# jzhangbs/MVSDF

Measured on AMD Instinct MI355X. Metric: traced rays/sec (fwd+bwd, 10 sphere iters, 4 src views), higher is better.
Workload: dtype f32x3

## Files before the change

mvsdf_amd/csrc/step_driver.hip:

```cpp
#include <hip/hip_runtime.h>
#include <stdint.h>
#include <stdlib.h>
#include <string.h>
#include <new>
#include "capi_util.h"
#include "step_internal.h"
#include <sched.h>
#include <time.h>

namespace {

inline size_t al256(size_t x) { return (x + 255) & ~(size_t)255; }

struct FwdOffsets {
    size_t w[MVSDF_STEP_MAX_LAYERS], wp[MVSDF_STEP_MAX_LAYERS], wpT[MVSDF_STEP_MAX_LAYERS], wp16[MVSDF_STEP_MAX_LAYERS];
    size_t wx3[MVSDF_STEP_MAX_LAYERS], wx3T[MVSDF_STEP_MAX_LAYERS];
    int chain_x3;
    size_t trace_ws, trace_ws_bytes;
    size_t inv, true_rows, true_rank, counts, view_sorted;
    size_t x_eval, y_eval, n_eval, sdf_ctx, rgb_sorted, render_ctx;
};
struct BwdOffsets {
    size_t dy, dn, dy_x, dn_x, din, drgb_sorted, render_ws, wsA, wsX, dx, fbar;
};

struct Step {
    MvsdfStepDesc d;
    MvsdfStepLayout lay;
    FwdOffsets fo;
    BwdOffsets bo;
    int R, E, M, Nout, K0r, nl;
    size_t woff[MVSDF_STEP_MAX_LAYERS], boff[MVSDF_STEP_MAX_LAYERS];
    size_t seg[2][3];
    long long* counts_host;
    long long* counts_host_dev;
    int can_defer;
    hipEvent_t ev_counts;
    bool counts_pending;
    long long counts_seq;
    hipStream_t counts_stream;
    int timing;
    hipEvent_t ev_t[9];
    bool timed, timed_bwd;
    hipStream_t side;
    hipEvent_t ev_fork, ev_join;
    int split_rows;
};

void make_descs(const Step& st, const MvsdfStepParams* prm, const char* fwd, MvsdfNetDesc* sdf, MvsdfNetDesc* sdfT, MvsdfNetDesc* rnd, MvsdfNetDesc* rndT) {
    const MvsdfStepDesc& d = st.d;
    auto fill = [&](MvsdfNetDesc* o, MvsdfNetDesc* oT, int l0, int n, bool is_sdf) {
        memset(o, 0, sizeof(*o));
        memset(oT, 0, sizeof(*oT));
        o->n_layers = oT->n_layers = n;
        for (int i = 0; i < n; ++i) {
            const int l = l0 + i;
            o->K[i] = d.K[l]; o->N[i] = d.N[l];
            oT->K[i] = d.N[l]; oT->N[i] = d.K[l];
            o->wp[i] = (const float*)(fwd + st.fo.wp[l]);
            oT->wp[i] = (const float*)(fwd + st.fo.wpT[l]);
            o->bias[i] = oT->bias[i] = prm->b[l];
            o->w[i] = oT->w[i] = (const float*)(fwd + st.fo.w[l]);
            if (is_sdf && d.trace_dtype != 0) o->wp16[i] = fwd + st.fo.wp16[l];
            if (is_sdf && st.fo.chain_x3) { o->wx3[i] = fwd + st.fo.wx3[l]; oT->wx3[i] = fwd + st.fo.wx3T[l]; }
        }
        if (is_sdf) {
            const unsigned m = d.skip_mask;
            const int single = (m && !(m & (m - 1))) ? __builtin_ctz(m) : -1;
            o->skip_layer = oT->skip_layer = m ? (single >= 0 ? single : __builtin_ctz(m)) : -1;
            o->skip_mask = (m && single < 0) ? m : 0;
            o->multires = oT->multires = d.multires;
            o->trace_dtype = (d.trace_dtype >= 1 && d.trace_dtype <= 5) ? d.trace_dtype : 0;
        } else {
            o->skip_layer = oT->skip_layer = -1;
        }
    };
    fill(sdf, sdfT, 0, d.n_sdf, true);
    fill(rnd, rndT, d.n_sdf, d.n_render, false);
}

__global__ void k_step_gather_x(const float* __restrict__ eik, int n_eik, const float* __restrict__ ds_on, const float* __restrict__ ds_jit, int n_ds,
                                const float* __restrict__ points, const long long* __restrict__ perm, int R, float* __restrict__ x_eval,
                                uint8_t* __restrict__ ones) {
    const int E = n_eik + 2 * n_ds, total = (E + R) * 3;
    for (int i = blockIdx.x * blockDim.x + threadIdx.x; i < total; i += gridDim.x * blockDim.x) {
        const int row = i / 3, c = i - 3 * row;
        float v;
        if (row < n_eik) v = eik[i];
        else if (row < n_eik + n_ds) v = ds_on[3 * (size_t)(row - n_eik) + c];
        else if (row < E) v = ds_jit[3 * (size_t)(row - n_eik - n_ds) + c];
        else v = points[3 * (size_t)perm[row - E] + c];
        x_eval[i] = v;
        if (ones && i < R) ones[i] = 1;
    }
}

__global__ void k_step_gather_drgb(const float* __restrict__ d_rgb, const long long* __restrict__ perm, int N, float* __restrict__ out) {
    const int i = blockIdx.x * blockDim.x + threadIdx.x;
    if (i >= 3 * N) return;
    const int row = i / 3, c = i - 3 * row;
    out[i] = d_rgb[3 * (size_t)perm[row] + c];
}

#define ST_TRY(expr) do { int rc_ = (expr); if (rc_) return rc_; } while (0)
#define ST_HIP(expr) do { hipError_t e_ = (expr); if (e_ != hipSuccess) return mv_check(e_, #expr); } while (0)

}

extern "C" {

int mvsdf_step_create(const MvsdfStepDesc* desc, MvsdfStepLayout* layout, void** out) {
    if (!desc || !layout || !out) return mv_fail(-1, "mvsdf_step_create: null argument");
    if (desc->trace_dtype == 1) return mv_fail(-2, "mvsdf_step_create: trace_dtype 1 (bf16 weights AND 8-bit activations) was removed in round 5: use 3 (bf16x2)");
    const MvsdfStepDesc& d = *desc;
    const int nl = d.n_sdf + d.n_render;
    if (d.B <= 0 || d.P <= 0 || d.n_eik < 0 || d.n_ds < 0 || d.n_sdf < 2 || d.n_render < 1 || d.n_sdf > MVSDF_MAX_LAYERS || d.n_render > MVSDF_MAX_LAYERS ||
        nl > MVSDF_STEP_MAX_LAYERS || (long long)d.B * d.P > (1ll << 24))
        return mv_fail(-1, "mvsdf_step_create: bad sizes");
    Step* st = new (std::nothrow) Step;
    if (!st) return mv_fail(-1, "mvsdf_step_create: out of host memory");
    memset(st, 0, sizeof(*st));
    st->d = d;
    st->R = d.B * d.P; st->E = d.n_eik + 2 * d.n_ds; st->M = st->R + st->E; st->nl = nl;
    st->Nout = d.N[d.n_sdf - 1]; st->K0r = d.K[d.n_sdf];
    st->split_rows = -1;
    const int R = st->R, M = st->M;
    MvsdfNetDesc sdf, sdfT, rnd, rndT;
    MvsdfStepParams fake;
    memset(&fake, 0, sizeof(fake));
    static const float dummy = 0.f;
    for (int l = 0; l < nl; ++l) fake.b[l] = &dummy;
    MvsdfStepLayout& L = st->lay;
    FwdOffsets& fo = st->fo;
    size_t p = 0;
    auto take = [&](size_t bytes) { const size_t o = p; p += al256(bytes ? bytes : 4); return o; };
    L.ray_dirs = take((size_t)R * 12); L.cam_loc = take((size_t)d.B * 12);
    L.points = take((size_t)R * 12); L.mask = take((size_t)R); L.dists = take((size_t)R * 4); L.counters = take(16 * 8);
    L.object_mask_out = take((size_t)R);
    fo.trace_ws_bytes = mvsdf_trace_workspace_bytes_n(R, d.tp.n_steps);
    fo.trace_ws = take(fo.trace_ws_bytes);
    fo.chain_x3 = mv_chain_x3_enabled();
    for (int l = 0; l < nl; ++l) {
        fo.w[l] = take((size_t)d.N[l] * d.K[l] * 4);
        fo.wp[l] = take(mvsdf_packed_floats(d.N[l], d.K[l]) * 4);
        fo.wpT[l] = take(mvsdf_packed_floats(d.K[l], d.N[l]) * 4);
        if (l < d.n_sdf && d.trace_dtype == 2) {
            fo.wp16[l] = take(mvsdf_packed_floats(d.N[l], d.K[l]) * 4);
        } else if (l < d.n_sdf && (d.trace_dtype == 3 || d.trace_dtype == 4)) {
            fo.wp16[l] = take(mvsdf_packed_bf16_bytes(d.N[l], d.K[l], 0));
        } else if (l < d.n_sdf && d.trace_dtype == 5) {
            fo.wp16[l] = take(3 * mvsdf_packed_bf16_bytes(d.N[l], d.K[l], 0));
        }
        if (l < d.n_sdf && fo.chain_x3) {
            fo.wx3[l] = d.trace_dtype == 5 ? fo.wp16[l] : take(3 * mvsdf_packed_bf16_bytes(d.N[l], d.K[l], 0));
            fo.wx3T[l] = take(3 * mvsdf_packed_bf16_bytes(d.K[l], d.N[l], 0));
        }
    }
    L.perm = take((size_t)R * 8); fo.inv = take((size_t)R * 8); fo.true_rows = take((size_t)R * 8); fo.true_rank = take((size_t)R * 4); fo.counts = take(4 * 8 + 4 * 4);
    fo.view_sorted = take((size_t)R * 12);
    fo.x_eval = take((size_t)M * 12); fo.y_eval = take((size_t)M * st->Nout * 4); fo.n_eval = take((size_t)M * 12);
    make_descs(*st, &fake, (const char*)nullptr, &sdf, &sdfT, &rnd, &rndT);
    for (int i = 0; i < d.n_sdf; ++i) { sdf.wp[i] = sdfT.wp[i] = &dummy; sdf.w[i] = &dummy; }
    for (int i = 0; i < d.n_render; ++i) { rnd.wp[i] = rndT.wp[i] = &dummy; }
    const size_t ctx_f = mvsdf_sdf_ctx_floats(&sdf, M, M), rctx_f = mvsdf_render_ctx_floats(&rnd, R);
    if (!ctx_f || !rctx_f) { delete st; return mv_fail(-2, "mvsdf_step_create: network descriptor rejected (layer dims / skip mask)"); }
    st->can_defer = (d.n_ds == 0 && mv_step_can_defer(&sdf, &sdfT, &rnd, &rndT)) ? 1 : 0;
    fo.sdf_ctx = take(ctx_f * 4);
    fo.rgb_sorted = take((size_t)R * 12);
    fo.render_ctx = take(rctx_f * 4);
    L.rgb_values = take((size_t)R * 12); L.sdf_output = take((size_t)R * 4); L.diff_pts = take((size_t)R * 12);
    L.eik_out = take((size_t)M * 4); L.points_hom = take((size_t)M * 16); L.grad_theta = take((size_t)M * 12);
    L.surf = take((size_t)(R + d.n_eik) * 4);
    L.fwd_bytes = p;
    BwdOffsets& bo = st->bo;
    p = 0;
    bo.dy = take((size_t)M * st->Nout * 4); bo.dn = take((size_t)M * 12);
    bo.dy_x = take((size_t)R * st->Nout * 4); bo.dn_x = take((size_t)R * 12);
    bo.din = take((size_t)R * st->K0r * 4); bo.drgb_sorted = take((size_t)R * 12);
    bo.render_ws = take(mvsdf_render_bwd_ws_floats(&rnd, R) * 4);
    bo.wsA = take(mvsdf_sdf_bwd_ws_floats(&sdf, M) * 4);
    bo.wsX = take(mvsdf_sdf_bwd_ws_floats(&sdf, R) * 4);
    bo.dx = take((size_t)R * 12); bo.fbar = take((size_t)R * 4);
    size_t off = 0;
    int lo = 0;
    const int cuts[2] = {d.n_sdf, nl};
    for (int net = 0; net < 2; ++net) {
        st->seg[net][0] = off;
        for (int l = lo; l < cuts[net]; ++l) { st->woff[l] = off; off += (size_t)d.N[l] * d.K[l]; }
        st->seg[net][1] = off;
        for (int l = lo; l < cuts[net]; ++l) { st->boff[l] = off; off += (size_t)d.N[l]; }
        st->seg[net][2] = off;
        lo = cuts[net];
    }
    L.dflat_floats = off;
    L.dflat = take(off * 4);
    L.bwd_bytes = p;
    *layout = L;
    *out = st;
    return 0;
}

void mvsdf_step_destroy(void* step) {
    Step* st = (Step*)step;
    if (!st) return;
    if (st->timing) for (int i = 0; i < 9; ++i) hipEventDestroy(st->ev_t[i]);
    if (st->counts_host) { hipEventDestroy(st->ev_counts); hipHostFree(st->counts_host); }
    if (st->side) { hipStreamSynchronize(st->side); hipEventDestroy(st->ev_fork); hipEventDestroy(st->ev_join); hipStreamDestroy(st->side); }
    delete st;
}

int mvsdf_step_set_timing(void* step, int enable) {
    Step* st = (Step*)step;
    if (!st) return mv_fail(-1, "mvsdf_step_set_timing: null step");
    if (enable && !st->timing) {
        for (int i = 0; i < 9; ++i) ST_HIP(hipEventCreate(&st->ev_t[i]));
        st->timing = 1;
    } else if (!enable && st->timing) {
        for (int i = 0; i < 9; ++i) hipEventDestroy(st->ev_t[i]);
        st->timing = 0;
    }
    st->timed = false; st->timed_bwd = false;
    return 0;
}

int mvsdf_step_trace_times(void* step, float ms[3]) {
    Step* st = (Step*)step;
    if (!st || !ms || !st->timing || !st->timed) return mv_fail(-1, "mvsdf_step_trace_times: timing is off or no forward has run");
    float a = 0.f, b = 0.f, c = 0.f;
    ST_HIP(hipEventElapsedTime(&a, st->ev_t[0], st->ev_t[1]));
    ST_HIP(hipEventElapsedTime(&b, st->ev_t[1], st->ev_t[2]));
    ST_HIP(hipEventElapsedTime(&c, st->ev_t[3], st->ev_t[4]));
    ms[0] = a; ms[1] = b; ms[2] = c;
    return 0;
}

int mvsdf_step_times(void* step, float ms[6]) {
    Step* st = (Step*)step;
    if (!st || !ms || !st->timing || !st->timed) return mv_fail(-1, "mvsdf_step_times: timing is off or no forward has run");
    if (int rc = mvsdf_step_trace_times(step, ms)) return rc;
    ST_HIP(hipEventElapsedTime(&ms[3], st->ev_t[4], st->ev_t[5]));
    ms[4] = 0.f;
    if (st->timed_bwd) ST_HIP(hipEventElapsedTime(&ms[4], st->ev_t[6], st->ev_t[7]));
    ST_HIP(hipEventElapsedTime(&ms[5], st->ev_t[8], st->ev_t[5]));
    return 0;
}

int mvsdf_step_forward(void* step, const MvsdfStepParams* prm, const MvsdfStepInputs* in, int d_mask, int e_mask, void* fwd_, void* stream) {
    Step* st = (Step*)step;
    if (!st || !prm || !in || !fwd_) return mv_fail(-1, "mvsdf_step_forward: null argument");
    const MvsdfStepDesc& d = st->d;
    if (!in->uv || !in->pose || !in->intrinsics || !in->object_mask || !in->object_mask_true || !in->intervals || !in->minsdf_steps ||
        (d.n_eik > 0 && !in->eik_points) || (d.n_ds > 0 && (!in->ds_on || !in->ds_jit || !in->ds_counts)))
        return mv_fail(-1, "mvsdf_step_forward: missing input");
    hipStream_t s = (hipStream_t)stream;
    if (!st->counts_host) {
        ST_HIP(hipHostMalloc((void**)&st->counts_host, MVSDF_STEP_COUNT_RING * 8 * sizeof(long long), hipHostMallocMapped | hipHostMallocCoherent));
        memset(st->counts_host, 0, MVSDF_STEP_COUNT_RING * 8 * sizeof(long long));
        if (hipHostGetDevicePointer((void**)&st->counts_host_dev, st->counts_host, 0) != hipSuccess) { (void)hipGetLastError(); st->counts_host_dev = nullptr; }
        if (hipEventCreateWithFlags(&st->ev_counts, hipEventDisableTiming) != hipSuccess) {
            hipHostFree(st->counts_host); st->counts_host = nullptr;
            return mv_fail(-1, "mvsdf_step_forward: hipEventCreate failed");
        }
    }
    char* fwd = (char*)fwd_;
    const MvsdfStepLayout& L = st->lay;
    const FwdOffsets& fo = st->fo;
    const int R = st->R, E = st->E, M = st->M, nl = st->nl;
    if (st->timing) ST_HIP(hipEventRecord(st->ev_t[8], s));
    float* w[MVSDF_STEP_MAX_LAYERS]; float* wp[MVSDF_STEP_MAX_LAYERS]; float* wpT[MVSDF_STEP_MAX_LAYERS];
    for (int l = 0; l < nl; ++l) { w[l] = (float*)(fwd + fo.w[l]); wp[l] = (float*)(fwd + fo.wp[l]); wpT[l] = (float*)(fwd + fo.wpT[l]); }
    float* ray_dirs = (float*)(fwd + L.ray_dirs); float* cam_loc = (float*)(fwd + L.cam_loc);
    {
        void* wp16[MVSDF_STEP_MAX_LAYERS]; int nsplit[MVSDF_STEP_MAX_LAYERS];
        void* wx3[MVSDF_STEP_MAX_LAYERS]; void* wx3T[MVSDF_STEP_MAX_LAYERS];
        for (int l = 0; l < nl; ++l) {
            const bool bf = l < d.n_sdf && d.trace_dtype != 0;
            wp16[l] = bf ? (void*)(fwd + fo.wp16[l]) : nullptr;
            const bool x3 = l < d.n_sdf && fo.chain_x3;
            wx3[l] = (x3 && d.trace_dtype != 5) ? (void*)(fwd + fo.wx3[l]) : nullptr;
            wx3T[l] = x3 ? (void*)(fwd + fo.wx3T[l]) : nullptr;
            nsplit[l] = 0;
        }
        const float* stage_dev = nullptr;
        if (in->host_stage) {
            if (hipHostGetDevicePointer((void**)&stage_dev, (void*)in->host_stage, 0) != hipSuccess || !stage_dev) {
                (void)hipGetLastError();
                return mv_fail(-1, "mvsdf_step_forward: host_stage is not device-visible pinned memory");
            }
        }
        ST_TRY(mv_step_prologue(nl, prm->v, prm->g, d.N, d.K, w, wp, wpT, wp16, nsplit, d.trace_dtype == 2 ? 1 : (d.trace_dtype == 5 ? 2 : 0), wx3, wx3T, in->uv, in->pose, in->intrinsics, d.B, d.P, ray_dirs, cam_loc,
                                (uint8_t*)(fwd + L.object_mask_out), (unsigned long long*)(fwd + L.counters), stage_dev, (float*)in->minsdf_steps, d.tp.n_steps,
                                (float*)in->eik_points, 3 * d.n_eik, stream));
    }
    MvsdfNetDesc sdf, sdfT, rnd, rndT;
    make_descs(*st, prm, fwd, &sdf, &sdfT, &rnd, &rndT);
    float* x_eval = (float*)(fwd + fo.x_eval); float* y_eval = (float*)(fwd + fo.y_eval); float* n_eval = (float*)(fwd + fo.n_eval);
    FwdGather g;
    g.eik = in->eik_points; g.on = in->ds_on; g.jit = in->ds_jit; g.pts = (float*)(fwd + L.points); g.perm = (long long*)(fwd + L.perm);
    g.n_eik = d.n_eik; g.n_ds = d.n_ds; g.x_out = x_eval;
    if (st->split_rows < 0) {
        const char* e = getenv("MVSDF_SPLIT_ROWS");
        st->split_rows = (e && *e) ? (atoi(e) != 0 && E >= 1) : mv_chain_split_pays(&sdf, E, M);
        if (st->split_rows) {
            int prio_least = 0, prio_greatest = 0;
            if (hipDeviceGetStreamPriorityRange(&prio_least, &prio_greatest) != hipSuccess) { (void)hipGetLastError(); prio_least = 0; }
            if (hipStreamCreateWithPriority(&st->side, hipStreamNonBlocking, prio_least) != hipSuccess) { (void)hipGetLastError(); st->side = nullptr; st->split_rows = 0; }
            else if (hipEventCreateWithFlags(&st->ev_fork, hipEventDisableTiming) != hipSuccess ||
                     hipEventCreateWithFlags(&st->ev_join, hipEventDisableTiming) != hipSuccess) {
                (void)hipGetLastError();
                if (st->ev_fork) { (void)hipEventDestroy(st->ev_fork); st->ev_fork = nullptr; }
                if (st->ev_join) { (void)hipEventDestroy(st->ev_join); st->ev_join = nullptr; }
                (void)hipStreamDestroy(st->side);
                st->side = nullptr; st->split_rows = 0;
            }
        }
    }
    bool split = st->split_rows == 1;
    struct SideGuard {
        hipStream_t side; bool armed;
        ~SideGuard() { if (armed && side) (void)hipStreamSynchronize(side); }
    } side_guard{st->side, false};
    if (split) ST_HIP(hipEventRecord(st->ev_fork, s));
    float* points = (float*)(fwd + L.points); uint8_t* mask = (uint8_t*)(fwd + L.mask); float* dists = (float*)(fwd + L.dists);
    unsigned long long* counters = (unsigned long long*)(fwd + L.counters);
    auto stage = [&](int which) {
        return mvsdf_trace_stage(which, &sdf, &d.tp, cam_loc, ray_dirs, in->object_mask, d.B, d.P, 1, in->intervals, in->minsdf_steps, points, mask, dists,
                                 counters, fwd + fo.trace_ws, fo.trace_ws_bytes, d.mt, d.mt_samples, stream);
    };
    if (st->timing) ST_HIP(hipEventRecord(st->ev_t[0], s));
    ST_TRY(mv_trace_stage1_prezeroed(&sdf, &d.tp, cam_loc, ray_dirs, in->object_mask, d.B, d.P, 1, in->intervals, in->minsdf_steps, points, mask, dists,
                                     counters, fwd + fo.trace_ws, fo.trace_ws_bytes, d.mt, d.mt_samples, stream));
    if (st->timing) ST_HIP(hipEventRecord(st->ev_t[1], s));
    if (split) {
        ST_HIP(hipStreamWaitEvent(st->side, st->ev_fork, 0));
        side_guard.armed = true;
        const int rcs = mv_sdf_forward_gather(&sdf, &sdfT, nullptr, &g, M, M, 0, E, y_eval, n_eval, (float*)(fwd + fo.sdf_ctx), st->side);
        if (rcs == 1) { split = false; side_guard.armed = false; }
        else if (rcs) return rcs;
        else ST_HIP(hipEventRecord(st->ev_join, st->side));
    }
    ST_TRY(stage(3));
    if (st->timing) ST_HIP(hipEventRecord(st->ev_t[2], s));
    long long* perm = (long long*)(fwd + L.perm); long long* inv = (long long*)(fwd + fo.inv); long long* true_rows = (long long*)(fwd + fo.true_rows);
    long long* counts = (long long*)(fwd + fo.counts); float* view_sorted = (float*)(fwd + fo.view_sorted);
    ST_TRY(mv_partition_rays_step(mask, d.use_object_mask ? in->object_mask : nullptr, in->object_mask_true, ray_dirs, R, perm, inv, true_rows, counts,
                                  view_sorted, (int*)(fwd + fo.true_rank), d.n_ds > 0 ? in->ds_counts : nullptr,
                                  st->counts_host_dev ? st->counts_host_dev + 8 * ((st->counts_seq + 1) % MVSDF_STEP_COUNT_RING) : nullptr, st->counts_seq + 1,
                                  (float*)(fwd + fo.counts + 32), d.n_eik, d.n_ds, d_mask, e_mask, stream));
    ++st->counts_seq;
    if (!st->counts_host_dev) {
        ST_HIP(hipMemcpyAsync(st->counts_host, counts, 4 * sizeof(long long), hipMemcpyDeviceToHost, s));
        ST_HIP(hipEventRecord(st->ev_counts, s));
    }
    st->counts_pending = true; st->counts_stream = s;
    if (st->timing) ST_HIP(hipEventRecord(st->ev_t[3], s));
    ST_TRY(stage(4));
    if (st->timing) { ST_HIP(hipEventRecord(st->ev_t[4], s)); st->timed = true; }
    {
        if (split) { ST_HIP(hipStreamWaitEvent(s, st->ev_join, 0)); side_guard.armed = false; }
        int rcf = mv_sdf_forward_gather(&sdf, &sdfT, nullptr, &g, M, M, split ? E : 0, M, y_eval, n_eval, (float*)(fwd + fo.sdf_ctx), stream);
        if (rcf == 1) {
            const int total = M * 3;
            hipLaunchKernelGGL(k_step_gather_x, dim3((total + 255) / 256), dim3(256), 0, s, in->eik_points, d.n_eik, in->ds_on, in->ds_jit, d.n_ds, points, perm,
                               R, x_eval, (uint8_t*)nullptr);
            ST_HIP(hipGetLastError());
            rcf = mvsdf_sdf_forward(&sdf, &sdfT, x_eval, M, M, y_eval, n_eval, (float*)(fwd + fo.sdf_ctx), stream);
        }
        if (rcf) return rcf;
    }
    float* rgb_sorted = (float*)(fwd + fo.rgb_sorted);
    ST_TRY(mvsdf_render_forward(&rnd, x_eval + 3 * (size_t)E, view_sorted, n_eval + 3 * (size_t)E, y_eval + (size_t)E * st->Nout + 2, st->Nout, R,
                                d.view_spec, rgb_sorted, (float*)(fwd + fo.render_ctx), stream));
    ST_TRY(mvsdf_step_outputs(R, d.n_eik, d.n_ds, st->Nout, counts, x_eval, y_eval, n_eval, inv, true_rows, rgb_sorted, d_mask, e_mask,
                              (float*)(fwd + L.rgb_values), (float*)(fwd + L.sdf_output), (float*)(fwd + L.diff_pts), (float*)(fwd + L.eik_out),
                              (float*)(fwd + L.points_hom), (float*)(fwd + L.grad_theta), (float*)(fwd + L.surf), stream));
    if (st->timing) ST_HIP(hipEventRecord(st->ev_t[5], s));
    return 0;
}

static int step_wait_seq(Step* st, long long seq, long long counts[4]) {
    long long* slot = st->counts_host + 8 * (seq % MVSDF_STEP_COUNT_RING);
    for (unsigned long long it = 1;; ++it) {
        const long long have = __atomic_load_n(&slot[4], __ATOMIC_ACQUIRE);
        if (have == seq) break;
        if (have > seq) return mv_fail(-4, "mvsdf_step_wait_counts_seq: the record of that forward was overwritten (read the counts from its forward block)");
        if (it < 5000) { __builtin_ia32_pause(); continue; }
        struct timespec ts = {0, 20000};
        nanosleep(&ts, nullptr);
        if ((it & 0x3ff) == 0 && seq == st->counts_seq) {
            const hipError_t q = hipStreamQuery(st->counts_stream);
            if (q == hipSuccess) {
                if (__atomic_load_n(&slot[4], __ATOMIC_ACQUIRE) == seq) break;
                return mv_fail(-1, "mvsdf_step_wait_counts: the forward finished without delivering its counts");
            }
            if (q != hipErrorNotReady) return mv_check(q, "mvsdf_step_wait_counts (hipStreamQuery)");
        }
    }
    for (int i = 0; i < 4; ++i) counts[i] = slot[i];
    if (__atomic_load_n(&slot[4], __ATOMIC_ACQUIRE) != seq) return mv_fail(-4, "mvsdf_step_wait_counts_seq: the record of that forward was overwritten (read the counts from its forward block)");
    return 0;
}

int mvsdf_step_wait_counts(void* step, long long counts[4]) {
    Step* st = (Step*)step;
    if (!st || !counts) return mv_fail(-1, "mvsdf_step_wait_counts: null argument");
    if (!st->counts_pending) return mv_fail(-1, "mvsdf_step_wait_counts: no forward is in flight");
    if (!st->counts_host_dev) {
        ST_HIP(hipEventSynchronize(st->ev_counts));
        for (int i = 0; i < 4; ++i) counts[i] = st->counts_host[i];
        st->counts_pending = false;
        return 0;
    }
    const int rc = step_wait_seq(st, st->counts_seq, counts);
    st->counts_pending = false;
    return rc;
}

long long mvsdf_step_seq(void* step) { return step ? ((Step*)step)->counts_seq : -1; }
size_t mvsdf_step_counts_offset(void* step) { return step ? ((Step*)step)->fo.counts : 0; }
int mvsdf_step_can_defer(void* step) { Step* st = (Step*)step; return (st && st->can_defer) ? 1 : 0; }
int mvsdf_step_saved_offsets(void* step, size_t out[6]) {
    Step* st = (Step*)step;
    if (!st || !out) return mv_fail(-1, "mvsdf_step_saved_offsets: null argument");
    out[0] = st->fo.x_eval; out[1] = st->fo.y_eval; out[2] = st->fo.n_eval; out[3] = st->fo.view_sorted; out[4] = st->fo.render_ctx; out[5] = st->fo.rgb_sorted;
    return 0;
}

int mvsdf_step_wait_counts_seq(void* step, long long seq, long long counts[4]) {
    Step* st = (Step*)step;
    if (!st || !counts) return mv_fail(-1, "mvsdf_step_wait_counts_seq: null argument");
    if (seq <= 0 || seq > st->counts_seq || !st->counts_host) return mv_fail(-1, "mvsdf_step_wait_counts_seq: no such forward");
    if (!st->counts_host_dev) {
        if (seq != st->counts_seq) return mv_fail(-4, "mvsdf_step_wait_counts_seq: the record of that forward was overwritten (read the counts from its forward block)");
        ST_HIP(hipEventSynchronize(st->ev_counts));
        for (int i = 0; i < 4; ++i) counts[i] = st->counts_host[i];
        return 0;
    }
    if (seq + MVSDF_STEP_COUNT_RING <= st->counts_seq) return mv_fail(-4, "mvsdf_step_wait_counts_seq: the record of that forward was overwritten (read the counts from its forward block)");
    const int rc = step_wait_seq(st, seq, counts);
    if (rc == 0 && seq == st->counts_seq) st->counts_pending = false;
    return rc;
}
// ... 139 lines not shown
```

mvsdf_amd/csrc/trace.hip:

```cpp
#include <stdlib.h>
#include <type_traits>
#include "tile_engine.h"
#include "tile_engine_bf16.h"
#include "tile_engine_bf16s.h"
#include "trace_params.h"
#include "capi_util.h"

struct RayCommon {
    float c[3], d[3];
};

__device__ __forceinline__ float mv_clamp(float v, float lo, float hi) { return v < lo ? lo : (v > hi ? hi : v); }

__device__ __forceinline__ bool mv_sphere_isect(const float* c, const float* d, float r, float& t0, float& t1) {
    const float dot = fmaf(d[2], c[2], fmaf(d[1], c[1], d[0] * c[0]));
    const float nrm = sqrtf(c[0] * c[0] + c[1] * c[1] + c[2] * c[2]);
    const float under = dot * dot - (nrm * nrm - r * r);
    const bool hit = under > 0.0f;
    float a = 0.0f, b = 0.0f;
    if (hit) {
        const float s = sqrtf(under);
        a = s * -1.0f - dot;
        b = s * 1.0f - dot;
    }
// ... 425 lines not shown
        const int kind = e >> 28;
        const bool om = kind & MV_ITEM_OM;
        cc = c.cam_loc + 3 * (gid / c.P);
        d = c.dirs + 3 * (size_t)gid;
        const float zmin = c.w_zmin[gid], zmax = c.w_zmax[gid];
        const int row = src ? src[it] : it;
        const float* sv = c.sv + (size_t)row * n_steps;
        if (mode == 0 && c.n_first < n_steps) {
            if (it == 0 && lead) {
                atomicAdd(&c.counters[MV_CNT_ROWS_SAMPLER], (unsigned long long)n_list * (unsigned long long)n_steps);
                atomicAdd(&c.counters[MV_CNT_ROWS_SAMPLER_EVAL], (unsigned long long)n_list * (unsigned long long)c.n_first);
            }
            const int ind = mv_first_where(sv, c.n_first, lane, 0);
            if (!(om && ind >= 1)) {
                cat = 1;
            } else if (lead) {
                dist = zmin + c.intervals[ind] * (zmax - zmin);
                have_dist = true;
                c.o_mask[gid] = 1;
                cat = 2;
                c.sec_state[gid] = zmin + c.intervals[ind - 1] * (zmax - zmin);
                c.sec_state[(size_t)c.R + gid] = dist;
                c.sec_state[2 * (size_t)c.R + gid] = sv[ind - 1];
                c.sec_state[3 * (size_t)c.R + gid] = sv[ind];
            }
        } else if (mode <= 1) {
            if (it == 0 && lead) {
                if (mode == 0) {
                    atomicAdd(&c.counters[MV_CNT_ROWS_SAMPLER], (unsigned long long)n_list * (unsigned long long)n_steps);
                    atomicAdd(&c.counters[MV_CNT_ROWS_SAMPLER_EVAL], (unsigned long long)n_list * (unsigned long long)n_steps);
                } else
                    atomicAdd(&c.counters[MV_CNT_ROWS_SAMPLER_EVAL], (unsigned long long)n_list * (unsigned long long)(n_steps - c.n_first));
            }
            int ind = mv_first_where(sv, n_steps, lane, 0);
            if (ind < 0) ind = mv_first_where(sv, n_steps, lane, 1);
            if (ind < 0) ind = n_steps - 1;
            const bool net_surf = sv[ind] < 0.f;
            const int i2 = (om && net_surf) ? 0 : mv_first_argmin(sv, n_steps, lane);
            if (lead) {
                dist = zmin + c.intervals[(om && net_surf) ? ind : i2] * (zmax - zmin);
                have_dist = true;
                c.o_mask[gid] = net_surf ? 1 : 0;
                const bool do_secant = c.training ? (net_surf && om) : net_surf;
                if (do_secant) {
                    int lo = ind - 1; if (lo < 0) lo += n_steps;
                    cat = 2;
                    c.sec_state[gid] = zmin + c.intervals[lo] * (zmax - zmin);
                    c.sec_state[(size_t)c.R + gid] = zmin + c.intervals[ind] * (zmax - zmin);
                    c.sec_state[2 * (size_t)c.R + gid] = sv[lo];
                    c.sec_state[3 * (size_t)c.R + gid] = sv[ind];
                }
            }
        } else {
            if (it == 0 && lead) atomicAdd(&c.counters[MV_CNT_ROWS_MINSDF], (unsigned long long)n_list * (unsigned long long)n_steps);
            const int bi = mv_first_argmin(sv, n_steps, lane);
            if (lead) { dist = c.steps[bi] * (zmax - zmin) + zmin; have_dist = true; }
        }
        if (lead && have_dist) {
            c.o_dists[gid] = dist;
            c.o_points[3 * (size_t)gid + 0] = cc[0] + dist * d[0];
            c.o_points[3 * (size_t)gid + 1] = cc[1] + dist * d[1];
            c.o_points[3 * (size_t)gid + 2] = cc[2] + dist * d[2];
        }
    }
    if (mode == 2) return;
    if (lead) s_cat[w] = cat;
    __syncthreads();
    if (threadIdx.x == 0) {
        unsigned n1 = 0, n2 = 0;
        for (int k = 0; k < MV_RED_WAVES; ++k) { n1 += s_cat[k] == 1; n2 += s_cat[k] == 2; }
        if (n1) s_base[0] = atomicAdd(&c.counters[MV_CNT_N_SAMPLER_REST], (unsigned long long)n1);
        if (n2) s_base[1] = atomicAdd(&c.counters[MV_CNT_N_SECANT], (unsigned long long)n2);
    }
    __syncthreads();
    if (lead && cat) {
        unsigned rank = 0;
        for (int k = 0; k < w; ++k) rank += s_cat[k] == cat;
        const unsigned long long k = s_base[cat - 1] + rank;
        if (cat == 1) { c.list_rest[k] = e; c.src_rest[k] = it; }
        else c.sec_list[k] = gid;
    }
}

template <int MT, int NTW, int NW, class NET>
__device__ void mv_secant_rays(const NET& net, const MvTraceParams& tp, const SampleCtx& c, int n_list, int block, float* smem) {
    constexpr int ROWS = 16 * MT;
    const int tid = threadIdx.x;
    const int r0 = block * ROWS;
    if (r0 >= n_list) return;
    const int n = min(ROWS, n_list - r0);
    TraceLds lds = mv_carve<NET>(smem, ROWS, net.S, 3 + 6 * net.multires, 0);
    const bool mine = tid < n;
    int gid = 0;
    float cc[3] = {0, 0, 0}, d[3] = {0, 0, 0}, z_low = 0, z_high = 0, sdf_low = 0, sdf_high = 1, z_pred = 0;
    if (mine) {
        gid = c.sec_list[r0 + tid];
        const int b = gid / c.P;
        for (int i = 0; i < 3; ++i) { cc[i] = c.cam_loc[3 * b + i]; d[i] = c.dirs[3 * (size_t)gid + i]; }
        z_low = c.sec_state[gid]; z_high = c.sec_state[(size_t)c.R + gid];
        sdf_low = c.sec_state[2 * (size_t)c.R + gid]; sdf_high = c.sec_state[3 * (size_t)c.R + gid];
        z_pred = -sdf_low * (z_high - z_low) / (sdf_high - sdf_low) + z_low;
    }
    for (int it = 0; it < tp.n_secant; ++it) {
        if (tid < ROWS) { float* p = lds.pts + tid * 3; p[0] = cc[0] + z_pred * d[0]; p[1] = cc[1] + z_pred * d[1]; p[2] = cc[2] + z_pred * d[2]; }
        __syncthreads();
        mv_eval_dispatch<MT, NTW, NW>(net, (n + 15) >> 4, lds.act, lds.pe, lds.pts, lds.sdfv, tid);
        if (mine) {
            const float sm = lds.sdfv[tid];
            if (sm > 0.f) { z_low = z_pred; sdf_low = sm; }
            if (sm < 0.f) { z_high = z_pred; sdf_high = sm; }
            z_pred = -sdf_low * (z_high - z_low) / (sdf_high - sdf_low) + z_low;
        }
    }
    if (mine) {
        c.o_dists[gid] = z_pred;
        c.o_points[3 * (size_t)gid + 0] = cc[0] + z_pred * d[0];
        c.o_points[3 * (size_t)gid + 1] = cc[1] + z_pred * d[1];
        c.o_points[3 * (size_t)gid + 2] = cc[2] + z_pred * d[2];
    }
    if (tid == 0) atomicAdd(&c.counters[MV_CNT_ROWS_SECANT], (unsigned long long)n * (unsigned long long)tp.n_secant);
}

template <class NET> struct mv_net_wt { static constexpr int v = 1; };
template <int NS, int WT> struct mv_net_wt<MvNetBs<NS, WT>> { static constexpr int v = WT; };
template <int MT, int NTW, int NW, class NET>
__global__ __launch_bounds__(64 * NW, (mv_net_wt<NET>::v == 3 && NTW == 2 && MT <= 2 && NW == 8) ? 4 : NW / 4) void k_ray_samples(NET net, MvTraceParams tp, SampleCtx c, RowSeg s0, RowSeg s1, int sec_blocks) {
    extern __shared__ __attribute__((aligned(16))) float smem[];
    int b = blockIdx.x;
    if (b < sec_blocks) {
        mv_secant_rays<(MT > 1 ? 1 : MT), NTW, NW, NET>(net, tp, c, (int)c.counters[MV_CNT_N_SECANT], b, smem);
        return;
    }
    b -= sec_blocks;
    const bool first = b < s0.blocks;
    if (!first && b - s0.blocks >= s1.blocks) return;
    const RowSeg sg = first ? s0 : s1;
    long long q0 = (long long)(first ? b : b - s0.blocks) * (16 * MT);
    const int n_list = (int)c.counters[sg.cnt_index];
    if (sg.unit_rows > 0) {
        if (q0 >= (long long)n_list * sg.ni + 16 * MT) return;
        __shared__ long long s_q0;
        if (threadIdx.x == 0) s_q0 = (long long)atomicAdd(&c.counters[MV_CNT_TAIL_NEXT], (unsigned long long)(16 * MT));
        __syncthreads();
        q0 = s_q0;
    }
    mv_eval_rows<MT, NTW, NW, NET>(net, tp, c, sg, q0, smem, n_list);
}
static int mv_tail_mode() {
    static int v = -1;
    if (v < 0) { const char* e = getenv("MVSDF_TAIL"); v = e ? atoi(e) : 1; }
    return v;
}
static unsigned* g_tail_probe = nullptr;
static unsigned* mv_tail_probe() { return g_tail_probe; }
extern "C" void mv_trace_set_tail_probe(unsigned* buf) { g_tail_probe = buf; }
static float* mv_minsdf_sv(float* ws, int R, int n_steps) {
    float* sec_state = ws + 2 * (size_t)R;
    int* w_list = (int*)(sec_state + 4 * (size_t)R);
    float* sv = (float*)(w_list + 3 * (size_t)R);
    int* list_rest = (int*)(sv + (size_t)R * n_steps);
    return (float*)(list_rest + 2 * (size_t)R);
}

static int mv_cu_count() {
    static int n = 0;
    if (n == 0) {
        int dev = 0, v = 0;
        if (hipGetDevice(&dev) != hipSuccess || hipDeviceGetAttribute(&v, hipDeviceAttributeMultiprocessorCount, dev) != hipSuccess || v <= 0) { (void)hipGetLastError(); v = 1; }
        n = v;
    }
    return n;
}
template <class NET>
static bool mv_tail_on(int training, const float* steps, int R, int mt1) {
    constexpr bool is_bf = !std::is_same<NET, MvNet>::value;
    const int grid1 = (R + 8 * mt1 - 1) / (8 * mt1);
    const int need = !is_bf ? 1 : ((mv_net_wt<NET>::v == 3 && R > 2048) ? 1 : 2);
    return training && steps && mv_tail_mode() >= need && grid1 <= mv_cu_count();
}

template <class NET>
static size_t trace_lds_bytes(const NET& net, int MT, int sv_floats, int rpw, bool sphere = false) {
    const int rows = 16 * MT, d0 = 3 + 6 * net.multires;
    size_t f = (size_t)mv_act_rows<NET>(rows, sphere) * net.S + ((rows * d0 + 3) & ~3) + rows * 4 + rows + sv_floats;
    return f * 4 + 16 + (size_t)rpw * (8 * 4 + 4) + 16;
}

template <int MT, int NTW, int NW, class NET>
static hipError_t launch_stage1(const NET& net, const MvTraceParams& tp, const float* cam_loc, const float* dirs, const uint8_t* om, int B, int P,
                                int training, const float* steps, int mt2, float* points, uint8_t* mask, float* dists, float* ws,
                                unsigned long long* counters, hipStream_t stream) {
    const int R = B * P, NR = 8 * MT;
    float* w_zmin = ws;
    float* w_zmax = w_zmin + R;
    int* w_list = (int*)(w_zmax + 5 * (size_t)R);
    int* w_list_min = w_list + R;
    TailCtx tail;
    memset(&tail, 0, sizeof(tail));
    const int grid1 = (R + NR - 1) / NR;
    if (mv_tail_on<NET>(training, steps, R, MT)) {
        tail.enable = 1;
        tail.steps = steps;
        tail.sv = mv_minsdf_sv(ws, R, tp.n_steps);
        tail.unit_rows = 16 * MT;
        tail.spin = 1;
        tail.probe = mv_tail_probe();
        static int stop_env = -1;
        if (stop_env < 0) { const char* e = mv_dev_env("MVSDF_TAIL_STOP"); stop_env = e ? atoi(e) : -1; }
        tail.stop_left = stop_env >= 0 ? stop_env : grid1 / 4;
    }
    const size_t lds1 = trace_lds_bytes(net, MT, 0, 0, NTW < 4);
    static size_t set1 = 0;
    if (lds1 > set1) {
        hipError_t e = hipFuncSetAttribute((const void*)k_sphere_trace<MT, NTW, NW, NET>, hipFuncAttributeMaxDynamicSharedMemorySize, (int)lds1);
        if (e != hipSuccess) return e;
        set1 = lds1;
    }
    hipLaunchKernelGGL((k_sphere_trace<MT, NTW, NW, NET>), dim3(grid1), dim3(64 * NW), lds1, stream, net, tp, cam_loc, dirs, om, R, P,
                       training, points, mask, dists, w_zmin, w_zmax, w_list, w_list_min, counters, tail);
    return hipGetLastError();
}

template <int MT, int NTW, int NW, class NET>
static hipError_t launch_stage2(const NET& net, const MvTraceParams& tp, const float* cam_loc, const float* dirs, int B, int P, int training,
                                const float* intervals, const float* steps, float* points, uint8_t* mask, float* dists, float* ws,
                                unsigned long long* counters, int parts, int mt1, hipStream_t stream) {
    const int R = B * P, ROWS = 16 * MT;
    float* w_zmin = ws;
    float* w_zmax = w_zmin + R;
    float* sec_state = w_zmax + R;
    int* w_list = (int*)(sec_state + 4 * (size_t)R);
    int* w_list_min = w_list + R;
    int* sec_list = w_list_min + R;
    float* sv = (float*)(sec_list + R);
    const size_t lds2 = trace_lds_bytes(net, MT, 0, 0);
    static size_t set2 = 0;
    if (lds2 > set2) {
        hipError_t e = hipFuncSetAttribute((const void*)k_ray_samples<MT, NTW, NW, NET>, hipFuncAttributeMaxDynamicSharedMemorySize, (int)lds2);
        if (e != hipSuccess) return e;
        set2 = lds2;
    }
    static int nf_env = -1;
    if (nf_env < 0) { const char* e = mv_dev_env("MVSDF_NFIRST"); nf_env = e ? atoi(e) : 12; if (nf_env < 2) nf_env = 2; }
    const int n = tp.n_steps, nf = nf_env < n ? nf_env : n;
    SampleCtx c;
    c.cam_loc = cam_loc; c.dirs = dirs; c.R = R; c.P = P; c.training = training; c.RPW = 0; c.intervals = intervals; c.steps = steps;
    c.o_points = points; c.o_mask = mask; c.o_dists = dists; c.w_zmin = w_zmin; c.w_zmax = w_zmax; c.sec_state = sec_state;
    c.sec_list = sec_list; c.sv = sv; c.counters = counters;
    c.list_rest = (int*)(sv + (size_t)R * n); c.src_rest = c.list_rest + R; c.n_first = nf;
    auto blocks_for = [&](int per_item) { return (int)(((long long)R * per_item + ROWS - 1) / ROWS); };
    const int sec_blocks = (R + 15) / 16, red_blocks = (R + MV_RED_WAVES - 1) / MV_RED_WAVES;
    const RowSeg none = {nullptr, nullptr, 0, 0, 1, 0, 0};
    if (parts & 1) {
        const RowSeg first = {w_list, nullptr, (int)MV_CNT_N_SAMPLER, 0, nf, blocks_for(nf), 0};
        hipLaunchKernelGGL((k_ray_samples<MT, NTW, NW, NET>), dim3(first.blocks), dim3(64 * NW), lds2, stream, net, tp, c, first, none, 0);
        hipLaunchKernelGGL(k_reduce_items, dim3(red_blocks), dim3(64 * MV_RED_WAVES), 0, stream, tp, c, w_list, (const int*)nullptr, (int)MV_CNT_N_SAMPLER, 0);
        if (nf < n) {
            const RowSeg rest = {c.list_rest, c.src_rest, (int)MV_CNT_N_SAMPLER_REST, nf, n - nf, blocks_for(n - nf), 0};
            hipLaunchKernelGGL((k_ray_samples<MT, NTW, NW, NET>), dim3(rest.blocks), dim3(64 * NW), lds2, stream, net, tp, c, rest, none, 0);
            hipLaunchKernelGGL(k_reduce_items, dim3(red_blocks), dim3(64 * MV_RED_WAVES), 0, stream, tp, c, c.list_rest, c.src_rest, (int)MV_CNT_N_SAMPLER_REST, 1);
        }
    }
    if (parts & 2) {
        const bool tail = mv_tail_on<NET>(training, steps, R, mt1);
        SampleCtx cm = c;
        if (tail) cm.sv = mv_minsdf_sv(ws, R, n);
        const RowSeg minsdf = {w_list_min, nullptr, (int)MV_CNT_N_MINSDF, 0, n, training ? blocks_for(n) + (tail ? 1 : 0) : 0, tail ? 1 : 0};
        hipLaunchKernelGGL((k_ray_samples<MT, NTW, NW, NET>), dim3(sec_blocks + minsdf.blocks), dim3(64 * NW), lds2, stream, net, tp, cm, minsdf, none,
                           sec_blocks);
        if (training) hipLaunchKernelGGL(k_reduce_items, dim3(red_blocks), dim3(64 * MV_RED_WAVES), 0, stream, tp, cm, w_list_min, (const int*)nullptr, (int)MV_CNT_N_MINSDF, 2);
    }
    if ((parts & 4) && training) {
        SampleCtx c2 = c;
        c2.sv = (float*)(c.src_rest + R);
        const bool tail = mv_tail_on<NET>(training, steps, R, mt1);
        const RowSeg minsdf = {w_list_min, nullptr, (int)MV_CNT_N_MINSDF, 0, n, blocks_for(n) + (tail ? 1 : 0), tail ? 1 : 0};
        hipLaunchKernelGGL((k_ray_samples<MT, NTW, NW, NET>), dim3(minsdf.blocks), dim3(64 * NW), lds2, stream, net, tp, c2, minsdf, none, 0);
        hipLaunchKernelGGL(k_reduce_items, dim3(red_blocks), dim3(64 * MV_RED_WAVES), 0, stream, tp, c2, w_list_min, (const int*)nullptr, (int)MV_CNT_N_MINSDF, 2);
    }
    if (parts & 8)
        hipLaunchKernelGGL((k_ray_samples<MT, NTW, NW, NET>), dim3(sec_blocks), dim3(64 * NW), lds2, stream, net, tp, c, none, none, sec_blocks);
    return hipGetLastError();
}

#ifndef MV_SPHERE_NW16
#define MV_SPHERE_NW16 1
#endif
template <class NET>
hipError_t mv_trace_launch(int stages, const NET& net, const MvTraceParams& tp, int mt1, int mt2, const float* cam_loc, const float* dirs,
                           const uint8_t* om, int B, int P, int training, const float* intervals, const float* steps, float* points,
                           uint8_t* mask, float* dists, float* ws, unsigned long long* counters, hipStream_t stream) {
    int maxnt = 0;
    for (int l = 0; l < net.n_layers - 1; ++l) maxnt = net.L[l].NT > maxnt ? net.L[l].NT : maxnt;
    if (maxnt > 32) return hipErrorInvalidValue;
    constexpr bool is_bf = !std::is_same<NET, MvNet>::value;
    const bool eight = is_bf || maxnt >= 16;
    const bool wide = maxnt > 16;
    hipError_t e = hipSuccess;
    auto eff = [&](int mt) { return wide ? (mt >= 2 ? 2 : 1) : (mt >= 4 ? 4 : (mt >= 2 ? 2 : 1)); };
    const int mt1_eff = eff(mt1), mt2_eff = eff(mt2);
#define MV_S1(MT_, NTW_, NW_) e = launch_stage1<MT_, NTW_, NW_>(net, tp, cam_loc, dirs, om, B, P, training, steps, mt2_eff, points, mask, dists, ws, counters, stream)
#define MV_S2(MT_, NTW_, NW_) e = launch_stage2<MT_, NTW_, NW_>(net, tp, cam_loc, dirs, B, P, training, intervals, steps, points, mask, dists, ws, counters, (stages >> 1) & 15, mt1_eff, stream)
    if (stages & 1) {
        if (eight) {
            if (wide) { if (mt1 >= 2) MV_S1(2, 4, 8); else MV_S1(1, 4, 8); }
            else if (mt1 >= 4) MV_S1(4, 2, 8); else if (mt1 >= 2) MV_S1(2, 2, 8);
            else {
                if constexpr (MV_SPHERE_NW16 != 0 && mv_net_wt<NET>::v == 3) MV_S1(1, 1, 16); else MV_S1(1, 2, 8);
            }
        } else if constexpr (!is_bf) {
            if (wide) { if (mt1 >= 2) MV_S1(2, 8, 4); else MV_S1(1, 8, 4); }
            else if (mt1 >= 4) MV_S1(4, 4, 4); else if (mt1 >= 2) MV_S1(2, 4, 4); else MV_S1(1, 4, 4);
        }
        if (e != hipSuccess) return e;
    }
    static int mtf_env = -1;
    if (mtf_env < 0) { const char* e2 = mv_dev_env("MVSDF_MT_FIRST"); mtf_env = e2 ? atoi(e2) : 0; }
    for (int part = 1; part <= 8; part <<= 1) {
        if (!((stages >> 1) & part)) continue;
        const int mtp = part == 1 ? (mtf_env > 0 ? mtf_env : (mv_net_wt<NET>::v == 3 ? (mt2 > 2 ? 2 : mt2) : ((long long)B * P <= 4096 ? 1 : mt2))) : mt2;
        const int st_ = stages;
        stages = (stages & 1) | (part << 1);
        if (eight) {
            if (wide) { if (mtp >= 2) MV_S2(2, 4, 8); else MV_S2(1, 4, 8); }
            else if (mtp >= 4) MV_S2(4, 2, 8); else if (mtp >= 2) MV_S2(2, 2, 8); else MV_S2(1, 2, 8);
        } else if constexpr (!is_bf) {
            if (wide) { if (mtp >= 2) MV_S2(2, 8, 4); else MV_S2(1, 8, 4); }
            else if (mtp >= 4) MV_S2(4, 4, 4); else if (mtp >= 2) MV_S2(2, 4, 4); else MV_S2(1, 4, 4);
        }
        stages = st_;
        if (e != hipSuccess) return e;
    }
#undef MV_S1
#undef MV_S2
    return e;
}

struct GenRay {
    float acc_s, acc_e, next_s, next_e, curr_s, curr_e, t0, t1, ts, te;
    int iters, k, phase, flags, pad0, pad1;
};

__device__ __forceinline__ void mv_gen_emit(const GenRay& g, const float* c, const float* d, uint8_t* req, float* pts) {
    const bool rs = g.flags & 4, re = g.flags & 8;
    req[0] = rs ? 1 : 0; req[1] = re ? 1 : 0;
    pts[0] = c[0] + g.ts * d[0]; pts[1] = c[1] + g.ts * d[1]; pts[2] = c[2] + g.ts * d[2];
    pts[3] = c[0] + g.te * d[0]; pts[4] = c[1] + g.te * d[1]; pts[5] = c[2] + g.te * d[2];
}

__global__ void k_gen_init(MvTraceParams tp, const float* __restrict__ cam_loc, const float* __restrict__ dirs, const uint8_t* __restrict__ om,
                           int R, int P, GenRay* __restrict__ state, uint8_t* __restrict__ req, float* __restrict__ pts) {
    const int gid = blockIdx.x * blockDim.x + threadIdx.x;
    if (gid >= R) return;
    float c[3], d[3];
    for (int i = 0; i < 3; ++i) { c[i] = cam_loc[3 * (gid / P) + i]; d[i] = dirs[3 * (size_t)gid + i]; }
    GenRay g;
    const bool isect = mv_sphere_isect(c, d, tp.r, g.t0, g.t1);
    g.acc_s = isect ? g.t0 : 0.f; g.acc_e = isect ? g.t1 : 0.f;
    g.next_s = g.next_e = g.curr_s = g.curr_e = 0.f;
    g.ts = g.acc_s; g.te = g.acc_e;
    g.iters = 0; g.k = 0; g.phase = isect ? 0 : 3;
    g.flags = (isect ? (1 | 2 | 4 | 8 | 16) : 0) | (om[gid] ? 32 : 0);
    g.pad0 = g.pad1 = 0;
    state[gid] = g;
    mv_gen_emit(g, c, d, req + 2 * (size_t)gid, pts + 6 * (size_t)gid);
}

__global__ void k_gen_step(MvTraceParams tp, const float* __restrict__ cam_loc, const float* __restrict__ dirs, int R, int P,
                           GenRay* __restrict__ state, const float* __restrict__ vals, uint8_t* __restrict__ req, float* __restrict__ pts,
                           unsigned long long* __restrict__ counters) {
    const int gid = blockIdx.x * blockDim.x + threadIdx.x;
    int nreq = 0;
    if (gid < R) {
        GenRay g = state[gid];
        if (g.phase != 3) {
            bool unf_s = g.flags & 1, unf_e = g.flags & 2;
            const bool req_s = g.flags & 4, req_e = g.flags & 8;
            nreq = (req_s ? 1 : 0) + (req_e ? 1 : 0);
            const float vs = req_s ? mv_clamp(vals[2 * (size_t)gid], -tp.dist_clip, tp.dist_clip) : 0.f;
            const float ve = req_e ? mv_clamp(vals[2 * (size_t)gid + 1], -tp.dist_clip, tp.dist_clip) : 0.f;
            bool nreq_s = false, nreq_e = false, end_iter = false;
            if (g.phase == 0) { g.next_s = vs; g.next_e = ve; }
            else if (g.phase == 1) { g.next_s = vs; g.next_e = ve; g.k = 0; }
            else { if (req_s) g.next_s = vs; if (req_e) g.next_e = ve; g.k++; }
            if (g.phase != 0) {
// ... 349 lines not shown
```

Before: 1.397 million.

## Add 16-wave secant kernel and optional side-stream minsdf overlap

Adds a dedicated secant-refinement kernel using 1024-thread blocks (16 waves) with an XR LDS carve for bf16x2 nets. It is enabled by default when the net is narrow. Separately, an env-gated option (off by default) runs the minsdf sample stage on a low-priority side stream so it overlaps with the secant and compaction work, joining before the SDF gather. The intent is to give the secant pass more parallel evaluation width and to hide minsdf latency, at the cost of larger LDS per block and extra stream/event management.

```diff
diff --git a/mvsdf_amd/csrc/step_driver.hip b/mvsdf_amd/csrc/step_driver.hip
--- a/mvsdf_amd/csrc/step_driver.hip
+++ b/mvsdf_amd/csrc/step_driver.hip
@@ -45,6 +45,9 @@
     hipStream_t side;
     hipEvent_t ev_fork, ev_join;
     int split_rows;
+    hipStream_t side_ms;
+    hipEvent_t ev_ms_fork, ev_ms_join;
+    int minsdf_side;
 };
 
 void make_descs(const Step& st, const MvsdfStepParams* prm, const char* fwd, MvsdfNetDesc* sdf, MvsdfNetDesc* sdfT, MvsdfNetDesc* rnd, MvsdfNetDesc* rndT) {
@@ -124,6 +127,7 @@
     st->R = d.B * d.P; st->E = d.n_eik + 2 * d.n_ds; st->M = st->R + st->E; st->nl = nl;
     st->Nout = d.N[d.n_sdf - 1]; st->K0r = d.K[d.n_sdf];
     st->split_rows = -1;
+    st->minsdf_side = -1;
     const int R = st->R, M = st->M;
     MvsdfNetDesc sdf, sdfT, rnd, rndT;
     MvsdfStepParams fake;
@@ -206,6 +210,7 @@
     if (st->timing) for (int i = 0; i < 9; ++i) hipEventDestroy(st->ev_t[i]);
     if (st->counts_host) { hipEventDestroy(st->ev_counts); hipHostFree(st->counts_host); }
     if (st->side) { hipStreamSynchronize(st->side); hipEventDestroy(st->ev_fork); hipEventDestroy(st->ev_join); hipStreamDestroy(st->side); }
+    if (st->side_ms) { hipStreamSynchronize(st->side_ms); hipEventDestroy(st->ev_ms_fork); hipEventDestroy(st->ev_ms_join); hipStreamDestroy(st->side_ms); }
     delete st;
 }
 
@@ -298,39 +303,58 @@
     FwdGather g;
     g.eik = in->eik_points; g.on = in->ds_on; g.jit = in->ds_jit; g.pts = (float*)(fwd + L.points); g.perm = (long long*)(fwd + L.perm);
     g.n_eik = d.n_eik; g.n_ds = d.n_ds; g.x_out = x_eval;
+    auto make_side = [](hipStream_t* side, hipEvent_t* fork, hipEvent_t* join) {
+        int prio_least = 0, prio_greatest = 0;
+        if (hipDeviceGetStreamPriorityRange(&prio_least, &prio_greatest) != hipSuccess) { (void)hipGetLastError(); prio_least = 0; }
+        if (hipStreamCreateWithPriority(side, hipStreamNonBlocking, prio_least) != hipSuccess) { (void)hipGetLastError(); *side = nullptr; return false; }
+        if (hipEventCreateWithFlags(fork, hipEventDisableTiming) != hipSuccess || hipEventCreateWithFlags(join, hipEventDisableTiming) != hipSuccess) {
+            (void)hipGetLastError();
+            if (*fork) { (void)hipEventDestroy(*fork); *fork = nullptr; }
+            if (*join) { (void)hipEventDestroy(*join); *join = nullptr; }
+            (void)hipStreamDestroy(*side);
+            *side = nullptr;
+            return false;
+        }
+        return true;
+    };
     if (st->split_rows < 0) {
         const char* e = getenv("MVSDF_SPLIT_ROWS");
         st->split_rows = (e && *e) ? (atoi(e) != 0 && E >= 1) : mv_chain_split_pays(&sdf, E, M);
-        if (st->split_rows) {
-            int prio_least = 0, prio_greatest = 0;
-            if (hipDeviceGetStreamPriorityRange(&prio_least, &prio_greatest) != hipSuccess) { (void)hipGetLastError(); prio_least = 0; }
-            if (hipStreamCreateWithPriority(&st->side, hipStreamNonBlocking, prio_least) != hipSuccess) { (void)hipGetLastError(); st->side = nullptr; st->split_rows = 0; }
-            else if (hipEventCreateWithFlags(&st->ev_fork, hipEventDisableTiming) != hipSuccess ||
-                     hipEventCreateWithFlags(&st->ev_join, hipEventDisableTiming) != hipSuccess) {
-                (void)hipGetLastError();
-                if (st->ev_fork) { (void)hipEventDestroy(st->ev_fork); st->ev_fork = nullptr; }
-                if (st->ev_join) { (void)hipEventDestroy(st->ev_join); st->ev_join = nullptr; }
-                (void)hipStreamDestroy(st->side);
-                st->side = nullptr; st->split_rows = 0;
-            }
-        }
+        if (st->split_rows && !make_side(&st->side, &st->ev_fork, &st->ev_join)) st->split_rows = 0;
+    }
+    if (st->minsdf_side < 0) {
+        const char* e = mv_dev_env("MVSDF_MINSDF_SIDE");
+        st->minsdf_side = (e && *e && atoi(e) >= 1 && atoi(e) <= 2) ? atoi(e) : 0;
+        if (st->minsdf_side && !make_side(&st->side_ms, &st->ev_ms_fork, &st->ev_ms_join)) st->minsdf_side = 0;
     }
     bool split = st->split_rows == 1;
+    const int ms_side = st->minsdf_side;
     struct SideGuard {
         hipStream_t side; bool armed;
         ~SideGuard() { if (armed && side) (void)hipStreamSynchronize(side); }
-    } side_guard{st->side, false};
+    } side_guard{st->side, false}, ms_guard{st->side_ms, false};
     if (split) ST_HIP(hipEventRecord(st->ev_fork, s));
     float* points = (float*)(fwd + L.points); uint8_t* mask = (uint8_t*)(fwd + L.mask); float* dists = (float*)(fwd + L.dists);
     unsigned long long* counters = (unsigned long long*)(fwd + L.counters);
-    auto stage = [&](int which) {
+    auto stage = [&](int which, void* strm) {
         return mvsdf_trace_stage(which, &sdf, &d.tp, cam_loc, ray_dirs, in->object_mask, d.B, d.P, 1, in->intervals, in->minsdf_steps, points, mask, dists,
-                                 counters, fwd + fo.trace_ws, fo.trace_ws_bytes, d.mt, d.mt_samples, stream);
+                                 counters, fwd + fo.trace_ws, fo.trace_ws_bytes, d.mt, d.mt_samples, strm);
     };
     if (st->timing) ST_HIP(hipEventRecord(st->ev_t[0], s));
     ST_TRY(mv_trace_stage1_prezeroed(&sdf, &d.tp, cam_loc, ray_dirs, in->object_mask, d.B, d.P, 1, in->intervals, in->minsdf_steps, points, mask, dists,
                                      counters, fwd + fo.trace_ws, fo.trace_ws_bytes, d.mt, d.mt_samples, stream));
     if (st->timing) ST_HIP(hipEventRecord(st->ev_t[1], s));
+    auto fork_minsdf = [&]() -> int {
+        ST_HIP(hipStreamWaitEvent(st->side_ms, st->ev_ms_fork, 0));
+        ms_guard.armed = true;
+        ST_TRY(stage(5, st->side_ms));
+        ST_HIP(hipEventRecord(st->ev_ms_join, st->side_ms));
+        return 0;
+    };
+    if (ms_side == 1) {
+        ST_HIP(hipEventRecord(st->ev_ms_fork, s));
+        ST_TRY(fork_minsdf());
+    }
     if (split) {
         ST_HIP(hipStreamWaitEvent(st->side, st->ev_fork, 0));
         side_guard.armed = true;
@@ -339,7 +363,7 @@
         else if (rcs) return rcs;
         else ST_HIP(hipEventRecord(st->ev_join, st->side));
     }
-    ST_TRY(stage(3));
+    ST_TRY(stage(3, stream));
     if (st->timing) ST_HIP(hipEventRecord(st->ev_t[2], s));
     long long* perm = (long long*)(fwd + L.perm); long long* inv = (long long*)(fwd + fo.inv); long long* true_rows = (long long*)(fwd + fo.true_rows);
     long long* counts = (long long*)(fwd + fo.counts); float* view_sorted = (float*)(fwd + fo.view_sorted);
@@ -354,10 +378,13 @@
     }
     st->counts_pending = true; st->counts_stream = s;
     if (st->timing) ST_HIP(hipEventRecord(st->ev_t[3], s));
-    ST_TRY(stage(4));
+    if (ms_side == 2) ST_HIP(hipEventRecord(st->ev_ms_fork, s));
+    ST_TRY(stage(ms_side ? 6 : 4, stream));
+    if (ms_side == 2) ST_TRY(fork_minsdf());
     if (st->timing) { ST_HIP(hipEventRecord(st->ev_t[4], s)); st->timed = true; }
     {
         if (split) { ST_HIP(hipStreamWaitEvent(s, st->ev_join, 0)); side_guard.armed = false; }
+        if (ms_side) { ST_HIP(hipStreamWaitEvent(s, st->ev_ms_join, 0)); ms_guard.armed = false; }
         int rcf = mv_sdf_forward_gather(&sdf, &sdfT, nullptr, &g, M, M, split ? E : 0, M, y_eval, n_eval, (float*)(fwd + fo.sdf_ctx), stream);
         if (rcf == 1) {
             const int total = M * 3;
diff --git a/mvsdf_amd/csrc/trace.hip b/mvsdf_amd/csrc/trace.hip
--- a/mvsdf_amd/csrc/trace.hip
+++ b/mvsdf_amd/csrc/trace.hip
@@ -531,14 +531,14 @@
     }
 }
 
-template <int MT, int NTW, int NW, class NET>
+template <int MT, int NTW, int NW, class NET, bool XR = false>
 __device__ void mv_secant_rays(const NET& net, const MvTraceParams& tp, const SampleCtx& c, int n_list, int block, float* smem) {
     constexpr int ROWS = 16 * MT;
     const int tid = threadIdx.x;
     const int r0 = block * ROWS;
     if (r0 >= n_list) return;
     const int n = min(ROWS, n_list - r0);
-    TraceLds lds = mv_carve<NET>(smem, ROWS, net.S, 3 + 6 * net.multires, 0);
+    TraceLds lds = mv_carve<NET, XR>(smem, ROWS, net.S, 3 + 6 * net.multires, 0);
     const bool mine = tid < n;
     int gid = 0;
     float cc[3] = {0, 0, 0}, d[3] = {0, 0, 0}, z_low = 0, z_high = 0, sdf_low = 0, sdf_high = 1, z_pred = 0;
@@ -553,7 +553,7 @@
     for (int it = 0; it < tp.n_secant; ++it) {
         if (tid < ROWS) { float* p = lds.pts + tid * 3; p[0] = cc[0] + z_pred * d[0]; p[1] = cc[1] + z_pred * d[1]; p[2] = cc[2] + z_pred * d[2]; }
         __syncthreads();
-        mv_eval_dispatch<MT, NTW, NW>(net, (n + 15) >> 4, lds.act, lds.pe, lds.pts, lds.sdfv, tid);
+        mv_eval_dispatch<MT, NTW, NW, NET, XR>(net, (n + 15) >> 4, lds.act, lds.pe, lds.pts, lds.sdfv, tid);
         if (mine) {
             const float sm = lds.sdfv[tid];
             if (sm > 0.f) { z_low = z_pred; sdf_low = sm; }
@@ -594,6 +594,11 @@
         q0 = s_q0;
     }
     mv_eval_rows<MT, NTW, NW, NET>(net, tp, c, sg, q0, smem, n_list);
+}
+template <class NET>
+__global__ __launch_bounds__(1024) void k_secant_rays16(NET net, MvTraceParams tp, SampleCtx c) {
+    extern __shared__ __attribute__((aligned(16))) float smem[];
+    mv_secant_rays<1, 1, 16, NET, true>(net, tp, c, (int)c.counters[MV_CNT_N_SECANT], blockIdx.x, smem);
 }
 static int mv_tail_mode() {
     static int v = -1;
@@ -673,7 +678,7 @@
 template <int MT, int NTW, int NW, class NET>
 static hipError_t launch_stage2(const NET& net, const MvTraceParams& tp, const float* cam_loc, const float* dirs, int B, int P, int training,
                                 const float* intervals, const float* steps, float* points, uint8_t* mask, float* dists, float* ws,
-                                unsigned long long* counters, int parts, int mt1, hipStream_t stream) {
+                                unsigned long long* counters, int parts, int mt1, bool sec16, hipStream_t stream) {
     const int R = B * P, ROWS = 16 * MT;
     float* w_zmin = ws;
     float* w_zmax = w_zmin + R;
@@ -727,14 +732,32 @@
         hipLaunchKernelGGL((k_ray_samples<MT, NTW, NW, NET>), dim3(minsdf.blocks), dim3(64 * NW), lds2, stream, net, tp, c2, minsdf, none, 0);
         hipLaunchKernelGGL(k_reduce_items, dim3(red_blocks), dim3(64 * MV_RED_WAVES), 0, stream, tp, c2, w_list_min, (const int*)nullptr, (int)MV_CNT_N_MINSDF, 2);
     }
-    if (parts & 8)
+    if (parts & 8) {
+        if constexpr (mv_net_wt<NET>::v == 3) {
+            if (sec16) {
+                const size_t lds16 = trace_lds_bytes(net, 1, 0, 0, true);
+                static size_t set16 = 0;
+                if (lds16 > set16) {
+                    hipError_t e = hipFuncSetAttribute((const void*)k_secant_rays16<NET>, hipFuncAttributeMaxDynamicSharedMemorySize, (int)lds16);
+                    if (e != hipSuccess) return e;
+                    set16 = lds16;
+                }
+                hipLaunchKernelGGL(k_secant_rays16<NET>, dim3(sec_blocks), dim3(1024), lds16, stream, net, tp, c);
+                return hipGetLastError();
+            }
+        }
         hipLaunchKernelGGL((k_ray_samples<MT, NTW, NW, NET>), dim3(sec_blocks), dim3(64 * NW), lds2, stream, net, tp, c, none, none, sec_blocks);
+    }
     return hipGetLastError();
 }
 
 #ifndef MV_SPHERE_NW16
 #define MV_SPHERE_NW16 1
 #endif
+static bool mv_secant_nw16_on() {
+    static const int v = [] { const char* e = mv_dev_env("MVSDF_SECANT_NW16"); return e ? atoi(e) : 1; }();
+    return v != 0;
+}
 template <class NET>
 hipError_t mv_trace_launch(int stages, const NET& net, const MvTraceParams& tp, int mt1, int mt2, const float* cam_loc, const float* dirs,
                            const uint8_t* om, int B, int P, int training, const float* intervals, const float* steps, float* points,
@@ -749,7 +772,8 @@
     auto eff = [&](int mt) { return wide ? (mt >= 2 ? 2 : 1) : (mt >= 4 ? 4 : (mt >= 2 ? 2 : 1)); };
     const int mt1_eff = eff(mt1), mt2_eff = eff(mt2);
 #define MV_S1(MT_, NTW_, NW_) e = launch_stage1<MT_, NTW_, NW_>(net, tp, cam_loc, dirs, om, B, P, training, steps, mt2_eff, points, mask, dists, ws, counters, stream)
-#define MV_S2(MT_, NTW_, NW_) e = launch_stage2<MT_, NTW_, NW_>(net, tp, cam_loc, dirs, B, P, training, intervals, steps, points, mask, dists, ws, counters, (stages >> 1) & 15, mt1_eff, stream)
+    const bool sec16 = eight && !wide && mv_secant_nw16_on();
+#define MV_S2(MT_, NTW_, NW_) e = launch_stage2<MT_, NTW_, NW_>(net, tp, cam_loc, dirs, B, P, training, intervals, steps, points, mask, dists, ws, counters, (stages >> 1) & 15, mt1_eff, sec16, stream)
     if (stages & 1) {
         if (eight) {
             if (wide) { if (mt1 >= 2) MV_S1(2, 4, 8); else MV_S1(1, 4, 8); }
```

Result: no change. 1.399 million, median of 4 (+0.2%).
